# 3dlg-hcvc/tricolo

Hardware: AMD Instinct MI355X
Metric: trimodal training samples/sec (32^3 voxel + 6-view) (higher is better)
Workload: dtype f16 (f16 activation storage + f16 MFMA operands, fp32 accumulate; bf16x3 heads/GRU; within 1e-3 of the fp32 reference)

## Files before the change

include/tricolo_hip.h:

```cpp
#ifndef TRICOLO_HIP_H
#define TRICOLO_HIP_H
#include <stddef.h>
#include <stdint.h>

#ifdef __cplusplus
extern "C" {
#endif

#define TRI_FMT_F32 0
#define TRI_FMT_BF16 1
#define TRI_FMT_F16 2

int tri_version(void);
const char* tri_last_error(void);

typedef struct TriConvDesc {
    int B, ID, IH, IW, Cin;
    int OD, OH, OW, Cout;
    int KD, KH, KW, stride, pad_d, pad_h, pad_w;
} TriConvDesc;

int tri_conv_kpad(int ntaps, int cin_stored);
typedef struct TriPrepDesc {
    const float* w;
    void* hi;
    void* lo;
    long s_row, s_tap, s_inner;
    int rows, ntaps, inner, inner_pad, kpad, fmt;
    int frag;
} TriPrepDesc;
int tri_weight_prep_multi(const TriPrepDesc* descs_dev, int n, void* stream);
int tri_weight_prep(const float* w, long s_row, long s_tap, long s_inner, int rows, int ntaps, int inner, int inner_pad,
                    void* w_hi, void* w_lo, int fmt, int frag, void* stream);

int tri_embedding_fwd(const int* tokens, const float* weight, int B, int L, int D, float* out, void* stream);
int tri_embedding_bwd(const int* tokens, const float* dout, int B, int L, int V, int D, int padding_idx, float* dweight, void* stream);

int tri_retrieval_topk(const float* text, const float* shape, const int* label, int Nq, int Ns, int D, int k, int* topk_idx ,
                       double* topk_sim , int* first_hit , void* stream);

int tri_linear_small_supported(int M, int K, int N);
int tri_linear_small_fwd(const float* x, const float* w, const float* bias, float* y, int M, int K, int N, int act, int split3, void* stream);
int tri_linear_small_dgrad(const float* dout, const float* y, const float* w, float* dx, int M, int K, int N, int act, int split3,
                           void* stream);
int tri_linear_small_wgrad(const float* x, const float* dout, const float* y, float* dw, float* db , int M, int K, int N,
                           int act, int split3, void* stream);
int tri_linear_small_bwd(const float* x, const float* dout, const float* y, const float* w, float* dx, float* dw, float* db, int M, int K,
                         int N, int act, int split3, void* stream);

int tri_conv_num_mtiles(const TriConvDesc* d, int split3);
int tri_conv_num_records(const TriConvDesc* d, int split3, int row_list);
int tri_conv_kernel_family(const TriConvDesc* d, int transposed, int split3);
int tri_conv_wgrad_kernel_family(const TriConvDesc* d, int act_fmt);
size_t tri_conv_workspace(const TriConvDesc* d, int transposed);
int tri_conv_fwd(const TriConvDesc* d, const void* in, const void* w_hi, const void* w_lo, void* out, const uint8_t* row_mask,
                 const float* bias, int act, int accumulate, float* stats, int act_fmt, void* workspace, size_t workspace_bytes,
                 const int* row_pos , const int* row_count ,
                 void* stream);
int tri_conv_dgrad(const TriConvDesc* d, const void* dout, const void* wt_hi, const void* wt_lo, void* din, const uint8_t* row_mask,
                   int accumulate, int act_fmt, void* workspace, size_t workspace_bytes,
                   const int* row_pos ,
                   const int* row_count ,
                   void* stream);
typedef struct TriConvBnSums {
    const void* y;
    const float* relu_scale;
    const float* relu_shift;
    const void* relu_out;
    float* partial;
} TriConvBnSums;
int tri_conv_dgrad_bn_records(const TriConvDesc* d, int accumulate, int act_fmt);
int tri_conv_dgrad_bn(const TriConvDesc* d, const void* dout, const void* wt_hi, const void* wt_lo, void* din, int accumulate,
                      int act_fmt, void* workspace, size_t workspace_bytes, const int* row_pos, const TriConvBnSums* sums, void* stream);
size_t tri_conv_wgrad_workspace(const TriConvDesc* d);
size_t tri_conv_plan_bytes(const TriConvDesc* d);
int tri_conv_plan_build(const TriConvDesc* d, void* plan, void* stream);
int tri_conv_wgrad(const TriConvDesc* d, const void* in, const void* dout, const uint8_t* row_mask, const void* plan ,
                   void* workspace, size_t workspace_bytes, float* dw, long s_co, long s_tap, long s_ci, int cin_real, int split3,
                   int act_fmt, float out_scale ,
                   const int* row_pos, const int* row_count ,
                   void* stream);
#ifndef TRI_WGRAD_GROUP_MAX
#define TRI_WGRAD_GROUP_MAX 24
#endif
typedef struct TriWgradReduce {
    const float* slab;
// ... 173 lines not shown
```

tricolo_amd/_C.py:

```python
from __future__ import annotations

import ctypes as C
import os

import torch

_HERE = os.path.dirname(os.path.abspath(__file__))
LIB_PATH = os.path.join(_HERE, "libtricolo_hip.so")


class TriConvDesc(C.Structure):
    _fields_ = [(n, C.c_int) for n in ("B", "ID", "IH", "IW", "Cin", "OD", "OH", "OW", "Cout",
                                       "KD", "KH", "KW", "stride", "pad_d", "pad_h", "pad_w")]


class TriPrepDesc(C.Structure):
    _fields_ = [("w", C.c_void_p), ("hi", C.c_void_p), ("lo", C.c_void_p), ("s_row", C.c_long), ("s_tap", C.c_long),
                ("s_inner", C.c_long), ("rows", C.c_int), ("ntaps", C.c_int), ("inner", C.c_int), ("inner_pad", C.c_int),
                ("kpad", C.c_int), ("fmt", C.c_int), ("frag", C.c_int)]


class TriWgradReduce(C.Structure):
    _fields_ = [("slab", C.c_void_p), ("dw", C.c_void_p), ("s_co", C.c_long), ("s_tap", C.c_long), ("s_ci", C.c_long)] + \
               [(n, C.c_int) for n in ("splits", "Cout", "Kpad", "ntaps", "cin_stored", "cin_real", "zlanes", "nblocks")] + \
# ... 5 lines not shown
                ("workspace_bytes", C.c_size_t), ("dw", C.c_void_p), ("s_co", C.c_long), ("s_tap", C.c_long), ("s_ci", C.c_long),
                ("cin_real", C.c_int), ("out_scale", C.c_float), ("row_pos", C.c_void_p), ("row_count", C.c_void_p)]


class TriConvBnSums(C.Structure):
    _fields_ = [("y", C.c_void_p), ("relu_scale", C.c_void_p), ("relu_shift", C.c_void_p), ("relu_out", C.c_void_p), ("partial", C.c_void_p)]


TRI_WGRAD_JOBS_MAX = 12
TRI_ERR_ARG, TRI_ERR_UNSUPPORTED = -1, -2

P, I, L, F, Z, DBL = C.c_void_p, C.c_int, C.c_long, C.c_float, C.c_size_t, C.c_double
DP = C.POINTER(TriConvDesc)

SIGNATURES = {
    "tri_version": (I, []),
    "tri_last_error": (C.c_char_p, []),
    "tri_conv_kpad": (I, [I, I]),
    "tri_weight_prep": (I, [P, L, L, L, I, I, I, I, P, P, I, I, P]),
    "tri_weight_prep_multi": (I, [P, I, P]),
    "tri_embedding_fwd": (I, [P, P, I, I, I, P, P]),
    "tri_embedding_bwd": (I, [P, P, I, I, I, I, I, P, P]),
    "tri_retrieval_topk": (I, [P, P, P, I, I, I, I, P, P, P, P]),
    "tri_linear_small_supported": (I, [I, I, I]),
    "tri_linear_small_fwd": (I, [P, P, P, P, I, I, I, I, I, P]),
    "tri_linear_small_dgrad": (I, [P, P, P, P, I, I, I, I, I, P]),
    "tri_linear_small_wgrad": (I, [P, P, P, P, P, I, I, I, I, I, P]),
    "tri_linear_small_bwd": (I, [P, P, P, P, P, P, P, I, I, I, I, I, P]),
    "tri_conv_num_mtiles": (I, [DP, I]),
    "tri_conv_num_records": (I, [DP, I, I]),
    "tri_conv_workspace": (Z, [DP, I]),
    "tri_conv_kernel_family": (I, [DP, I, I]),
    "tri_conv_wgrad_kernel_family": (I, [DP, I]),
    "tri_conv_fwd": (I, [DP, P, P, P, P, P, P, I, I, P, I, P, Z, P, P, P]),
    "tri_conv_dgrad": (I, [DP, P, P, P, P, P, I, I, P, Z, P, P, P]),
    "tri_conv_dgrad_bn_records": (I, [DP, I, I]),
    "tri_conv_dgrad_bn": (I, [DP, P, P, P, P, I, I, P, Z, P, C.POINTER(TriConvBnSums), P]),
    "tri_conv_wgrad_workspace": (Z, [DP]),
    "tri_conv_plan_bytes": (Z, [DP]),
    "tri_conv_plan_build": (I, [DP, P, P]),
    "tri_conv_wgrad": (I, [DP, P, P, P, P, P, Z, P, L, L, L, I, I, I, F, P, P, P]),
    "tri_conv_wgrad_partial": (I, [DP, P, P, P, P, P, Z, P, L, L, L, I, I, I, F, P, P, P, P]),
    "tri_wgrad_reduce_grouped": (I, [P, I, P]),
    "tri_wgrad_reduce_grouped_noted": (I, [P, I, P, P]),
    "tri_conv_stem_wgrad_bn": (I, [DP, P, P, P, P, P, P, P, P, P, P, Z, P, L, L, L, I, I, F, P, P]),
    "tri_conv_wgrad_group_info": (I, [DP, I, P, P, P]),
    "tri_conv_wgrad_partial_group": (I, [P, I, I, P, P]),
    "tri_bn_finalize": (I, [P, I, I, P, I, P, P, P, P, P, F, F, P, P, P, P, P]),
    "tri_bn_eval_coeffs": (I, [I, P, P, P, P, F, P, P, P, P, P]),
    "tri_bn_act": (I, [P, P, P, P, P, P, P, L, I, I, I, P]),
    "tri_relu_bwd": (I, [P, P, P, L, I, P]),
    "tri_bn_bwd_num_blocks": (I, [L]),
    "tri_bn_bwd_reduce": (I, [P, P, L, I, P, P, P, P, P, I, P]),
    "tri_bn_bwd_finalize": (I, [P, I, I, P, I, P, P, P, P, P, P, P, P, F, P]),
    "tri_bn_bwd_small": (I, [P, P, L, I, P, I, P, P, P, P, P, P, P, P, I, P, P, P, F, I, P]),
    "tri_bn_bwd_apply": (I, [P, P, P, P, P, P, P, L, I, P, P, P, P, I, I, P]),
    "tri_bn_bwd_pair_reduce": (I, [P, P, P, P, L, I, P, P, I, P]),
    "tri_bn_bwd_pair_finalize": (I, [P, P, I, I, I, P, P, P, P, P, P, P, P, F, P]),
    "tri_bn_bwd_pair_apply": (I, [P, P, P, P, P, P, P, P, P, L, I, I, P]),
    "tri_bn_relu_pool3d_fwd": (I, [P, P, P, P, I, I, I, P, P, I, P]),
    "tri_pool3d_bwd_route": (I, [P, P, P, P, P, P, I, I, I, P, I, P]),
    "tri_pool3d_bwd_route_rows": (I, [P, P, P, P, P, P, I, I, I, P, P, P, I, P]),
    "tri_pool3d_bwd_route_rows_num_blocks": (I, [I, I, I]),
    "tri_pool3d_bwd_route_rows_reduce": (I, [P, P, P, P, P, P, I, I, I, P, P, P, P, I, P]),
    "tri_bn_bwd_apply_rows": (I, [P, P, P, P, P, P, I, P, P, L, I, P]),
    "tri_bn_bwd_rows_scratch": (C.c_size_t, [I]),
# ... 129 lines not shown
```

tricolo_amd/csrc/conv_wgrad.hip:

```cpp
#include "common.h"
#include <stdio.h>
#include <stdlib.h>
#include "../../include/tricolo_hip.h"
#include "conv_vox.h"

struct WgradArgs {
    const void* in;
    const void* dout;
    const uint8_t* row_mask;
    const int* row_pos;
    const int* row_count;
    float* slab;
    const int* plan_off;
    const unsigned* plan_mask;
    unsigned in_bytes;
    int B, ID, IH, IW, Cin;
    int OD, OH, OW, Cout;
    int KD, KH, KW, stride, pd, ph, pw;
    int Kpad, M, ntaps, cin_shift, steps_per_split, ntiles, nsplits;
    int plan_ring;
    FastDiv dOW, dOH, dOD, dCin;
#ifdef WGRAD_STAMPS
    long long* dbg;
#endif
// ... 889 lines not shown
                const int p0 = pc0 + toff, p1 = pc1 + toff;
                s16x4 lo = __builtin_amdgcn_ds_read_tr16_b64_v4i16((s16x4 __attribute__((address_space(3)))*)(slab + p0 * 128 + ((cq ^ (p0 & 3)) << 5) + fp * 8));
                s16x4 hi = __builtin_amdgcn_ds_read_tr16_b64_v4i16((s16x4 __attribute__((address_space(3)))*)(slab + p1 * 128 + ((cq ^ (p1 & 3)) << 5) + fp * 8));
                typedef short s16x8 __attribute__((ext_vector_type(8)));
                const s16x8 rr = {lo[0], lo[1], lo[2], lo[3], hi[0], hi[1], hi[2], hi[3]};
                const v8 bf = __builtin_bit_cast(v8, rr);
#pragma unroll
                for (int ct = 0; ct < 4; ++ct) acc[j][ct] = MM::mma(af[ct], bf, acc[j][ct]);
            }
            xx0 += 32; while (xx0 >= W) { xx0 -= W; ++rr0; }
            xx1 += 32; while (xx1 >= W) { xx1 -= W; ++rr1; }
        }
    }
    float* out = p.slab + (size_t)blockIdx.x * 64 * 576;
#pragma unroll
    for (int j = 0; j < 9; ++j) {
        const int nt = wave + 4 * j;
        const int k0 = (nt >> 2) * 64 + (nt & 3) * 16;
#pragma unroll
        for (int ct = 0; ct < 4; ++ct)
#pragma unroll
            for (int r = 0; r < 4; ++r) out[(size_t)(ct * 16 + fg * 4 + r) * 576 + k0 + fr] = acc[j][ct][r];
    }
}

struct KrowArgs {
    const void* in; const void* dout; float* slab;
    unsigned in_bytes, dout_bytes;
    int NH, H, W, Cin, Cout, Kpad;
    int Hin, Win;
    int rps, P, npiece;
    int nsteps, steps_per_split, nsplits, ntiles, ci_chunks;
    FastDiv dH, dP, dW;
};
struct KrowJobs {
    KrowArgs d[WGRAD_JOBS_MAX];
    int first_block[WGRAD_JOBS_MAX + 1];
    int n;
};
static_assert(sizeof(KrowJobs) <= 4096, "the job table travels in the kernel arguments (4 KB)");
#define KROW_SLAB_PX 96
#define KROW_SLAB_PX_S2 160
__device__ __forceinline__ int krow_sw(int r, int xs, int W) {
    const int hb = W > 8 ? (xs >> 3) & 1 : (W > 4 ? r & 1 : (r >> 1) & 1);
    return ((xs >> 1) & 1) | (hb << 1);
}
template <int CO_T, typename E, int S = 1>
__global__ __launch_bounds__(256, 2) void conv_wgrad_krow_kernel(const KrowJobs jobs) {
    typedef Mma<E> MM;
    typedef typename MM::v8 v8;
    constexpr int KB = 64;
    constexpr int XROW = CO_T * 2, X_BYTES = KB * XROW;
    constexpr int SLAB_BYTES = (S == 1 ? KROW_SLAB_PX : KROW_SLAB_PX_S2) * 128, STAGE = X_BYTES + SLAB_BYTES;
    constexpr int NSP = SLAB_BYTES / 4096;
    constexpr int XRPI = 1024 / XROW, XNI = KB / (4 * XRPI);
    constexpr int TM = CO_T / 32;
    static_assert((4 * XRPI) % 16 == 0 && XNI >= 1, "lane -> chunk map must not depend on the instruction");
    extern __shared__ __attribute__((aligned(16))) char smem[];
    int ji = 0;
    while (ji + 1 < jobs.n && (int)blockIdx.x >= jobs.first_block[ji + 1]) ++ji;
    const KrowArgs& p = jobs.d[ji];
    const int bid = (int)blockIdx.x - jobs.first_block[ji];
    const int t = threadIdx.x, lane = t & 63, wave = __builtin_amdgcn_readfirstlane(t >> 6);
    const int ntiles = p.ntiles;
    int split, tile;
    if (p.nsplits >= 16) {
        const int grp = bid / (8 * ntiles), rem = bid - grp * 8 * ntiles;
        split = grp * 8 + (rem & 7);
        tile = rem >> 3;
    } else {
        const int nb = p.nsplits * ntiles;
        if (bid >= nb) return;
        const int lid = xcd_remap(bid, nb);
        split = lid / ntiles;
        tile = lid - split * ntiles;
    }
    if (split >= p.nsplits) return;
    const int ky = tile % 3, rest = tile / 3;
    const int cic = rest % p.ci_chunks, cot = rest / p.ci_chunks;
    const int co0 = cot * CO_T, ci0 = cic * 64;
    const int ks_begin = split * p.steps_per_split, ks_end = min(p.nsteps, ks_begin + p.steps_per_split);
    const int W = p.W, P = p.P, H = p.H, Cin = p.Cin, Cout = p.Cout;
    const int st = S ? S : (p.Hin != p.H ? 2 : 1);
    const int wi = wave >> 1, wj = wave & 1;
    const int fr = lane & 15, fg = lane >> 4, fqq = fr >> 2, fp = fr & 3;

    const int xrow0 = wave * XRPI + lane / (XROW / 16), xsl = lane % (XROW / 16);
    const int xchunk = ((((xsl >> 1) ^ nat_sw<XROW>(xrow0)) & (XROW / 32 - 1)) << 1) | (xsl & 1);
    const unsigned xoff = (unsigned)((xrow0 * Cout + co0 + xchunk * 8) * 2);
    const unsigned xstep = (unsigned)(4 * XRPI * Cout * 2);
    const unsigned step_bytes = (unsigned)(p.rps * W) * (unsigned)(Cout * 2);
    int s_r[NSP], s_col[NSP];
#pragma unroll
    for (int i = 0; i < NSP; ++i) {
        const int pi = wave + 4 * i;
// ... 72 lines not shown
        }
    };

    if (ks_begin < ks_end) {
        issue_x(ks_begin, 0);
        issue_slab(ks_begin, 0);
        int buf = 0;
        for (int ks = ks_begin; ks < ks_end; ++ks) {
            asm volatile("s_waitcnt vmcnt(0)" ::: "memory");
            __builtin_amdgcn_s_barrier();
            asm volatile("" ::: "memory");
            const bool more = ks + 1 < ks_end;
            if (more) issue_x(ks + 1, buf ^ 1);
#pragma unroll
            for (int h = 0; h < 2; ++h) {
                if (h == 1 && more) issue_slab(ks + 1, buf ^ 1);
                compute(buf, h);
            }
            buf ^= 1;
        }
    }
    float* slab = p.slab + (size_t)split * Cout * p.Kpad;
#pragma unroll
    for (int a = 0; a < TM; ++a)
#pragma unroll
        for (int r = 0; r < 4; ++r) {
            const int co = co0 + wi * (CO_T / 2) + a * 16 + fg * 4 + r;
#pragma unroll
            for (int b = 0; b < 6; ++b) {
                const int tt = 6 * wj + b, kx = tt >> 2, cq = tt & 3;
                slab[(size_t)co * p.Kpad + (ky * 3 + kx) * Cin + ci0 + cq * 16 + fr] = acc[a][b][r];
            }
        }
}

__device__ __forceinline__ unsigned wgrad_nonfinite(float x) { return (__float_as_uint(x) & 0x7f800000u) == 0x7f800000u ? 1u : 0u; }
__device__ __forceinline__ void wgrad_note_bad(unsigned bad, int* note) {
    if (note && __any(bad) && (threadIdx.x & 63) == 0) atomicMax(note + 2, note[0] + note[3] + 1);
}
__device__ __forceinline__ void wgrad_reduce_block(const float* __restrict__ slab, int splits, int Cout, int Kpad, int ntaps, int cin_stored,
                                                   int cin_real, float* __restrict__ dw, long s_co, long s_tap, long s_ci, int zlanes,
                                                   float out_scale, unsigned block, float4* part, unsigned& bad, int kw_real = 0,
                                                   int kw_shift = 3) {
    const int kq = 256 / zlanes;
    const int ql = threadIdx.x % kq, zl = threadIdx.x / kq;
    const int K4 = (ntaps * cin_stored) >> 2;
    const long quad = (long)block * kq + ql;
    const bool live = quad < (long)Cout * K4;
    const int co = live ? (int)(quad / K4) : 0, k = live ? (int)(quad - (long)co * K4) * 4 : 0;
    float4 s = make_float4(0.f, 0.f, 0.f, 0.f);
    if (live) {
        const float* src = slab + (size_t)co * Kpad + k;
        const size_t zs = (size_t)Cout * Kpad;
#pragma unroll 4
        for (int z = zl; z < splits; z += zlanes) {
            float4 v = *(const float4*)(src + z * zs);
            s.x += v.x; s.y += v.y; s.z += v.z; s.w += v.w;
        }
    }
    part[threadIdx.x] = s;
    __syncthreads();
    if (zl == 0 && live) {
        for (int z = 1; z < zlanes; ++z) {
            float4 v = part[z * kq + ql];
            s.x += v.x; s.y += v.y; s.z += v.z; s.w += v.w;
        }
// ... 215 lines not shown
    static int per_cu = -1;
    if (per_cu < 0) per_cu = 2;
    *grid = tri_internal_num_cus() * (per_cu < 1 ? 1 : per_cu);
    if (*grid > g->ntiles) *grid = g->ntiles;
    return true;
}

static bool krow_geometry(const TriConvDesc* d, int act_fmt, KrowArgs* g, int* co_t, int* tiles, int* steps) {
    if (!act_fmt || krow_wgrad_disabled()) return false;
    if (d->KD != 1 || d->ID != 1 || d->KH != 3 || d->KW != 3 || (d->stride != 1 && d->stride != 2) || d->pad_d != 0 || d->pad_h != 1 || d->pad_w != 1) return false;
    if (d->Cin % 64 || d->Cout % 64 || d->OH * d->stride != d->IH || d->OW * d->stride != d->IW) return false;
    const int W = d->OW, H = d->OH;
    if (W < 4 || W > 64) return false;
    const size_t in_bytes = (size_t)d->B * d->IH * d->IW * d->Cin * 2, dout_bytes = (size_t)d->B * H * W * d->Cout * 2;
    if (in_bytes >= ((size_t)1 << 31) || dout_bytes >= ((size_t)1 << 31)) return false;
    KrowArgs a{};
    a.in_bytes = (unsigned)in_bytes; a.dout_bytes = (unsigned)dout_bytes;
    a.NH = d->B * H; a.H = H; a.W = W; a.Cin = d->Cin; a.Cout = d->Cout; a.Kpad = 9 * d->Cin;
    a.Hin = d->IH; a.Win = d->IW;
    a.rps = 64 / W;
    a.P = d->stride == 1 ? ((W + 3) & ~1) : 2 * W + 2;
    if (a.rps * a.P > (d->stride == 1 ? KROW_SLAB_PX : KROW_SLAB_PX_S2)) return false;
    a.npiece = (a.rps * a.P + 7) / 8;
    a.nsteps = (a.NH + a.rps - 1) / a.rps;
    a.ci_chunks = d->Cin / 64;
    *co_t = d->Cout % 128 == 0 ? 128 : 64;
    a.ntiles = (d->Cout / *co_t) * 3 * a.ci_chunks;
    a.dH = make_fastdiv(H); a.dP = make_fastdiv(a.P); a.dW = make_fastdiv(W);
    *g = a;
    *tiles = a.ntiles;
    *steps = a.nsteps;
    return true;
}
#define KROW_TARGET_BLOCKS 512
static void krow_plan_alone(int tiles, int steps, int* sps, int* splits) {
    int s = KROW_TARGET_BLOCKS / tiles;
    const int max_by_steps = steps / 4 > 0 ? steps / 4 : 1;
    if (s > max_by_steps) s = max_by_steps;
    if (s < 1) s = 1;
    if (s > 1024) s = 1024;
    *sps = (steps + s - 1) / s;
    *splits = (steps + *sps - 1) / *sps;
}
static inline int krow_blocks(const KrowArgs& a) {
    return a.nsplits >= 16 ? ((a.nsplits + 7) / 8) * 8 * a.ntiles : (a.nsplits * a.ntiles + 7) / 8 * 8;
}
template <int CO_T, typename E, int S>
static int launch_krow_jobs(const KrowArgs* a, int n, hipStream_t stream) {
    constexpr int STAGE = 64 * CO_T * 2 + (S == 1 ? KROW_SLAB_PX : KROW_SLAB_PX_S2) * 128;
    KrowJobs jobs{};
    int order[WGRAD_JOBS_MAX];
    for (int i = 0; i < n; ++i) order[i] = i;
    for (int i = 1; i < n; ++i)
        for (int j = i; j > 0 && a[order[j]].steps_per_split > a[order[j - 1]].steps_per_split; --j) { int t = order[j]; order[j] = order[j - 1]; order[j - 1] = t; }
    int blocks = 0;
    for (int i = 0; i < n; ++i) {
        jobs.d[i] = a[order[i]];
        jobs.first_block[i] = blocks;
        blocks += krow_blocks(a[order[i]]);
    }
    jobs.first_block[n] = blocks;
    jobs.n = n;
    static bool attr_set = false;
    if (!attr_set) {
        hipFuncSetAttribute((const void*)conv_wgrad_krow_kernel<CO_T, E, S>, hipFuncAttributeMaxDynamicSharedMemorySize, 2 * STAGE);
        attr_set = true;
    }
    conv_wgrad_krow_kernel<CO_T, E, S><<<dim3(blocks), 256, 2 * STAGE, stream>>>(jobs);
    return tri_check_launch("tri_conv_wgrad(krow)");
}
static int launch_krow(int co_t, int act_fmt, const KrowArgs* a, int n, hipStream_t s) {
    int n2 = 0;
    for (int i = 0; i < n; ++i) n2 += a[i].Hin != a[i].H;
    if (n2 && n2 != n) {
#define TRI_KR0 (act_fmt == TRI_FMT_F16 ? (co_t == 128 ? launch_krow_jobs<128, f16_t, 0>(a, n, s) : launch_krow_jobs<64, f16_t, 0>(a, n, s))   \
                                        : (co_t == 128 ? launch_krow_jobs<128, bf16_t, 0>(a, n, s) : launch_krow_jobs<64, bf16_t, 0>(a, n, s)))
        return TRI_KR0;
#undef TRI_KR0
    }
    const bool s2 = n2 > 0;
#define TRI_KR(S_)                                                                                                                      \
    (act_fmt == TRI_FMT_F16 ? (co_t == 128 ? launch_krow_jobs<128, f16_t, S_>(a, n, s) : launch_krow_jobs<64, f16_t, S_>(a, n, s))      \
                            : (co_t == 128 ? launch_krow_jobs<128, bf16_t, S_>(a, n, s) : launch_krow_jobs<64, bf16_t, S_>(a, n, s)))
    return s2 ? TRI_KR(2) : TRI_KR(1);
#undef TRI_KR
}

extern "C" size_t tri_conv_wgrad_workspace(const TriConvDesc* d) {
    size_t need = 0;
    {
        StemWgradArgs sg; int grid;
        if (stem_wgrad_geometry(d, 1, &sg, &grid)) need = (size_t)grid * 64 * d->KH * 32 * sizeof(float);
        C64WgradArgs cg;
        if (c64_wgrad_geometry(d, 1, &cg, &grid)) need = (size_t)grid * 64 * 576 * sizeof(float);
        TriVox0Geom vg;
        if (tri_internal_vox0_geometry(d->B, d->ID, d->IH, d->IW, d->Cin, d->OD, d->OH, d->OW, d->Cout, d->KD, d->KH, d->KW, d->stride, d->pad_d,
                                       d->pad_h, d->pad_w, &vg) && tri_internal_vox0_wgrad_grid(vg) > 0)
            need = (size_t)tri_internal_vox0_wgrad_grid(vg) * 32 * 144 * sizeof(float);
        KrowArgs kg; int co_t, tiles, steps;
        if (krow_geometry(d, 1, &kg, &co_t, &tiles, &steps)) {
            int sps, splits;
            krow_plan_alone(tiles, steps, &sps, &splits);
            const size_t n = (size_t)splits * d->Cout * kg.Kpad * sizeof(float);
            if (n > need) need = n;
        }
    }
    for (int mode = 0; mode < 4; ++mode) {
        int BI, BJ, tiles, splits, sps, Kpad, dma;
        wgrad_plan(d, mode & 1, mode >> 1, &BI, &BJ, &tiles, &splits, &sps, &Kpad, &dma);
        size_t n = (size_t)splits * d->Cout * Kpad * sizeof(float);
        if (n > need) need = n;
    }
    return need;
}

extern "C" int tri_conv_wgrad_kernel_family(const TriConvDesc* d, int act_fmt) {
    {
        TriVox0Geom vg;
        if (act_fmt && tri_internal_vox0_geometry(d->B, d->ID, d->IH, d->IW, d->Cin, d->OD, d->OH, d->OW, d->Cout, d->KD, d->KH, d->KW, d->stride,
                                                  d->pad_d, d->pad_h, d->pad_w, &vg) && tri_internal_vox0_wgrad_grid(vg) > 0)
            return 6;
    }
    {
        C64WgradArgs cg; KrowArgs kg; int grid, co_t, tiles, steps;
        if (!c64_wgrad_geometry(d, act_fmt, &cg, &grid) && krow_geometry(d, act_fmt, &kg, &co_t, &tiles, &steps)) return 7;
    }
    int BI, BJ, tiles, splits, sps, Kpad, dma;
    wgrad_plan(d, act_fmt, 0, &BI, &BJ, &tiles, &splits, &sps, &Kpad, &dma);
    return dma ? 2 : 0;
}

static inline int wgrad_dma_blocks(const WgradArgs& a) {
    return a.nsplits >= 16 ? ((a.nsplits + 7) / 8) * 8 * a.ntiles : a.nsplits * a.ntiles;
}
static inline size_t wgrad_dma_plan_bytes(const WgradArgs& a) {
    const size_t entries = a.plan_ring ? (size_t)2 * WGRAD_RING_STEPS * 64 : (size_t)a.steps_per_split * 64;
    return entries * (a.row_count ? 12 : 8);
}
template <int BI, int BJ, typename E, int NWI = 2, int NWJ = 2>
static int launch_wgrad_dma_jobs(const WgradArgs* a, int n, hipStream_t stream) {
    constexpr int STAGE = 64 * (BI * 2 + BJ * 2);
    WgradJobs jobs{};
    size_t plan_bytes = 0;
    int blocks = 0;
    for (int i = 0; i < n; ++i) {
        jobs.d[i] = a[i];
#ifdef WGRAD_STAMPS
        jobs.d[i].dbg = g_wgrad_dbg;
#endif
        jobs.first_block[i] = blocks;
        blocks += wgrad_dma_blocks(a[i]);
        if (wgrad_dma_plan_bytes(a[i]) > plan_bytes) plan_bytes = wgrad_dma_plan_bytes(a[i]);
    }
    jobs.first_block[n] = blocks;
    jobs.n = n;
    size_t smem = 2 * STAGE + 512 + plan_bytes;
#ifdef WGRAD_STAMPS
    smem += 2048;
#endif
    static bool attr_set = false;
    if (!attr_set) {
        hipFuncSetAttribute((const void*)conv_wgrad_dma_kernel<BI, BJ, E, NWI, NWJ>, hipFuncAttributeMaxDynamicSharedMemorySize,
// ... 167 lines not shown
    {
        TriVox0Geom vg; int grid;
        if (row_mask && !row_count && !split3 && act_fmt &&
            tri_internal_vox0_geometry(d->B, d->ID, d->IH, d->IW, d->Cin, d->OD, d->OH, d->OW, d->Cout, d->KD, d->KH, d->KW, d->stride, d->pad_d,
                                       d->pad_h, d->pad_w, &vg) && (grid = tri_internal_vox0_wgrad_grid(vg)) > 0) {
            const size_t need = (size_t)grid * 32 * 144 * sizeof(float);
            if (workspace_bytes < need) { tri_set_error("wgrad(vox0): workspace too small"); return TRI_ERR_ARG; }
            int rc = tri_internal_vox0_wgrad_launch(vg, grid, d->B, in, dout, row_mask, (float*)workspace, act_fmt, (hipStream_t)stream);
            if (rc) return rc;
            const long quads = (long)32 * 36;
            int zlanes = 1;
            while (zlanes < 64 && zlanes * 2 <= grid && quads * zlanes < 262144) zlanes *= 2;
            const int kq = 256 / zlanes;
            pending->slab = (const float*)workspace; pending->dw = dw; pending->s_co = s_co; pending->s_tap = s_tap; pending->s_ci = s_ci;
            pending->splits = grid; pending->Cout = 32; pending->Kpad = 144; pending->ntaps = 36; pending->cin_stored = 4;
            pending->cin_real = cin_real; pending->zlanes = zlanes; pending->nblocks = (int)((quads + kq - 1) / kq);
            pending->out_scale = out_scale; pending->kw_real = 3; pending->kw_shift = 2;
            return 0;
        }
    }
    {
        StemWgradArgs sg; int grid;
        if (!row_mask && !row_count && !split3 && stem_wgrad_geometry(d, act_fmt, &sg, &grid)) {
            sg.in = in; sg.dout = dout;
            sg.y = nullptr;
            return stem_wgrad_launch(d, sg, grid, workspace, workspace_bytes, dw, s_co, s_tap, s_ci, cin_real, act_fmt, out_scale, pending, stream);
        }
    }
    if (d->Cin % 4 != 0 || d->Cout % 4 != 0) { tri_set_error("wgrad: channels must be multiples of 4"); return TRI_ERR_ARG; }
    {
        KrowArgs kg; int co_t, tiles, steps;
        if (!row_mask && !row_count && !split3 && krow_geometry(d, act_fmt, &kg, &co_t, &tiles, &steps)) {
            int sps, splits;
            krow_plan_alone(tiles, steps, &sps, &splits);
            if (workspace_bytes < (size_t)splits * d->Cout * kg.Kpad * sizeof(float)) { tri_set_error("wgrad(krow): workspace too small"); return TRI_ERR_ARG; }
            kg.in = in; kg.dout = dout; kg.slab = (float*)workspace; kg.steps_per_split = sps; kg.nsplits = splits;
            int rc = launch_krow(co_t, act_fmt, &kg, 1, (hipStream_t)stream);
            if (rc) return rc;
            wgrad_fill_pending(d, (const float*)workspace, splits, kg.Kpad, dw, s_co, s_tap, s_ci, cin_real, out_scale, pending);
            return 0;
        }
    }
    int BI, BJ, tiles, splits, sps, Kpad, dma;
    wgrad_plan(d, act_fmt, row_count != nullptr, &BI, &BJ, &tiles, &splits, &sps, &Kpad, &dma);
    if (workspace_bytes < (size_t)splits * d->Cout * Kpad * sizeof(float)) { tri_set_error("wgrad: workspace too small"); return TRI_ERR_ARG; }
    WgradArgs a{};
    {
        int rc = wgrad_fill_args(d, in, dout, row_mask, plan, (float*)workspace, row_pos, row_count, split3, act_fmt, Kpad, sps, tiles, splits, &a);
        if (rc) return rc;
    }
    hipStream_t s = (hipStream_t)stream;
    int rc;
#define TRI_WG(BI_, BJ_)                                                                                   \
    (act_fmt == TRI_FMT_F16 ? launch_wgrad<BI_, BJ_, 1, f16_t>(a, tiles, splits, s)                      \
     : act_fmt == TRI_FMT_BF16 ? launch_wgrad<BI_, BJ_, 1, bf16_t>(a, tiles, splits, s)                  \
              : (split3 ? launch_wgrad<BI_, BJ_, 2, float>(a, tiles, splits, s) : launch_wgrad<BI_, BJ_, 1, float>(a, tiles, splits, s)))
    if (dma) {
        if ((size_t)a.M * a.Cout * 2 >= ((size_t)1 << 31)) { tri_set_error("wgrad: dOut tensor >= 2 GiB (32-bit buffer offsets)"); return TRI_ERR_UNSUPPORTED; }
        if (act_fmt == TRI_FMT_F16) rc = BI == 128 ? launch_wgrad_dma<128, 128, f16_t>(a, tiles, splits, s) : launch_wgrad_dma<64, 128, f16_t>(a, tiles, splits, s);
        else rc = BI == 128 ? launch_wgrad_dma<128, 128, bf16_t>(a, tiles, splits, s) : launch_wgrad_dma<64, 128, bf16_t>(a, tiles, splits, s);
    } else if (BI == 128) rc = TRI_WG(128, 128);
    else if (BJ == 256) rc = TRI_WG(64, 256);
    else rc = TRI_WG(64, 128);
#undef TRI_WG
    if (rc) return rc;
    wgrad_fill_pending(d, (const float*)workspace, splits, Kpad, dw, s_co, s_tap, s_ci, cin_real, out_scale, pending);
    return 0;
}

static bool wgrad_wide_tiles() {
// ... 17 lines not shown
        KrowArgs kg; int co_t;
        if (krow_geometry(d, act_fmt, &kg, &co_t, tiles, steps)) { *family = co_t == 128 ? 4 : (d->stride == 2 ? 7 : 5); return 0; }
    }
    int BI, BJ, t, splits, sps, Kpad, dma;
    wgrad_plan(d, act_fmt, 0, &BI, &BJ, &t, &splits, &sps, &Kpad, &dma);
    if (!dma) return 0;
    *family = BI == 128 ? 1 : 2;
    if (BI == 128 && d->Cout % 256 == 0 && wgrad_wide_tiles()) {
        *family = 3;
        t = (d->Cout / 256) * ((Kpad + 127) / 128);
    }
    *tiles = t;
    *steps = (int)(((long)d->B * d->OD * d->OH * d->OW + 63) / 64);
    return 0;
}
extern "C" int tri_conv_wgrad_partial_group(const TriWgradJob* jobs, int n, int act_fmt, TriWgradReduce* pending, void* stream) {
    if (n < 1 || n > WGRAD_JOBS_MAX || !jobs || !pending) { tri_set_error("wgrad group: 1..TRI_WGRAD_JOBS_MAX jobs"); return TRI_ERR_ARG; }
    static_assert(WGRAD_JOBS_MAX == TRI_WGRAD_JOBS_MAX, "header and kernel disagree");
    {
        int fam, t0, st0;
        tri_conv_wgrad_group_info(jobs[0].d, act_fmt, &fam, &t0, &st0);
        if (fam >= 4 && fam <= 7) {
            KrowArgs ka[WGRAD_JOBS_MAX];
            int co_t0 = 0, tl[WGRAD_JOBS_MAX], st[WGRAD_JOBS_MAX];
            long total = 0;
            for (int i = 0; i < n; ++i) {
                int co_t;
                if (jobs[i].row_pos || jobs[i].row_count || !krow_geometry(jobs[i].d, act_fmt, &ka[i], &co_t, &tl[i], &st[i]) || (i && co_t != co_t0)) {
                    tri_set_error("wgrad group: jobs must share one groupable kernel family"); return TRI_ERR_ARG;
                }
                co_t0 = co_t;
                total += (long)tl[i] * st[i];
            }
            int common = (int)((total + wgrad_group_target(fam) - 1) / wgrad_group_target(fam));
            if (common < 8) common = 8;
            for (int i = 0; i < n; ++i) {
                int sps_alone, splits_alone;
                krow_plan_alone(tl[i], st[i], &sps_alone, &splits_alone);
                int sps = n == 1 ? sps_alone : (common > sps_alone ? common : sps_alone);
                if (sps > st[i]) sps = st[i];
                const int splits = (st[i] + sps - 1) / sps;
                sps = (st[i] + splits - 1) / splits;
                const TriConvDesc* d = jobs[i].d;
                if (jobs[i].workspace_bytes < (size_t)splits * d->Cout * ka[i].Kpad * sizeof(float)) { tri_set_error("wgrad group(krow): workspace too small"); return TRI_ERR_ARG; }
                ka[i].in = jobs[i].in; ka[i].dout = jobs[i].dout; ka[i].slab = (float*)jobs[i].workspace;
                ka[i].steps_per_split = sps; ka[i].nsplits = splits;
                wgrad_fill_pending(d, (const float*)jobs[i].workspace, splits, ka[i].Kpad, jobs[i].dw, jobs[i].s_co, jobs[i].s_tap, jobs[i].s_ci,
                                   jobs[i].cin_real, jobs[i].out_scale, &pending[i]);
            }
            return launch_krow(co_t0, act_fmt, ka, n, (hipStream_t)stream);
        }
    }
    WgradArgs a[WGRAD_JOBS_MAX];
    int fam0 = 0, ind_sps[WGRAD_JOBS_MAX], tiles[WGRAD_JOBS_MAX], steps[WGRAD_JOBS_MAX], Kpads[WGRAD_JOBS_MAX];
    long total = 0;
    for (int i = 0; i < n; ++i) {
        int fam;
        tri_conv_wgrad_group_info(jobs[i].d, act_fmt, &fam, &tiles[i], &steps[i]);
        if (!fam || (i && fam != fam0)) { tri_set_error("wgrad group: jobs must share one groupable kernel family"); return TRI_ERR_ARG; }
        fam0 = fam;
        int BI, BJ, t, splits, dma;
        wgrad_plan(jobs[i].d, act_fmt, 0, &BI, &BJ, &t, &splits, &ind_sps[i], &Kpads[i], &dma);
        total += (long)tiles[i] * steps[i];
    }
    const int target = wgrad_group_target(fam0);
    int common = (int)((total + target - 1) / target);
    if (common < 1) common = 1;
    for (;; ++common) {
        long wgs = 0;
        for (int i = 0; i < n; ++i) {
            const int sps = common > ind_sps[i] ? common : ind_sps[i];
            wgs += (long)tiles[i] * ((steps[i] + sps - 1) / sps);
        }
        if (wgs <= target || common >= 4096) break;
    }
    for (int i = 0; i < n; ++i) {
        int sps = (n == 1 && fam0 != 3) ? ind_sps[i] : (common > ind_sps[i] ? common : ind_sps[i]);
        if (sps > steps[i]) sps = steps[i];
        const int splits = (steps[i] + sps - 1) / sps;
        if (n > 1 || fam0 == 3) sps = (steps[i] + splits - 1) / splits;
        const TriConvDesc* d = jobs[i].d;
        if (jobs[i].workspace_bytes < (size_t)splits * d->Cout * Kpads[i] * sizeof(float)) { tri_set_error("wgrad group: workspace too small"); return TRI_ERR_ARG; }
        if ((size_t)d->B * d->OD * d->OH * d->OW * d->Cout * 2 >= ((size_t)1 << 31)) { tri_set_error("wgrad: dOut tensor >= 2 GiB (32-bit buffer offsets)"); return TRI_ERR_UNSUPPORTED; }
// ... 51 lines not shown
```

tricolo_amd/ops.py:

```python
from __future__ import annotations

import math
import os

import torch

from . import _C
from ._C import check, lib, make_desc, ptr, stream

_PRECISIONS = ("bf16", "bf16x3", "f16")
_FMT = {torch.float32: 0, torch.bfloat16: 1, torch.float16: 2}
F16_GRAD_SCALE = float(os.environ.get("TRICOLO_F16_GRAD_SCALE", "4096"))
if not (F16_GRAD_SCALE >= 1.0 and math.frexp(F16_GRAD_SCALE)[0] == 0.5):
    raise ValueError(f"TRICOLO_F16_GRAD_SCALE={F16_GRAD_SCALE!r}: must be a power of two >= 1 (the kernels divide it out exactly)")
_default_precision = os.environ.get("TRICOLO_PRECISION", "bf16x3")


def set_default_precision(p: str):
    global _default_precision
    if p not in _PRECISIONS:
        raise ValueError(f"precision must be one of {_PRECISIONS}")
    _default_precision = p


# ... 145 lines not shown
    return 1 if lo is not None else (2 if x.dtype != torch.float32 else 0)


_FRAG_FAMILIES = (13, 14, 15)


class ConvGeom:

    def __init__(self, B, in_grid, cin, cin_stored, cout, kernel, stride, pad, weight_strides):
        ID, IH, IW = in_grid
        KD, KH, KW = kernel
        pd, ph, pw = pad
        OD = (ID + 2 * pd - KD) // stride + 1
        OH = (IH + 2 * ph - KH) // stride + 1
        OW = (IW + 2 * pw - KW) // stride + 1
        self.B, self.in_grid, self.out_grid = B, (ID, IH, IW), (OD, OH, OW)
        self.cin, self.cin_stored, self.cout = cin, cin_stored, cout
        self.kernel, self.stride, self.pad = kernel, stride, pad
        self.ntaps = KD * KH * KW
        self.strides = weight_strides
        self.desc = make_desc(B, ID, IH, IW, cin_stored, OD, OH, OW, cout, KD, KH, KW, stride, pd, ph, pw)
        self.kpad = lib().tri_conv_kpad(self.ntaps, cin_stored)
        self.kpad_t = lib().tri_conv_kpad(self.ntaps, cout)
        self.M = B * OD * OH * OW
        self.M_in = B * ID * IH * IW
        self.num_mtiles = {m: lib().tri_conv_num_mtiles(_C.C.byref(self.desc), m) for m in (0, 1, 2)}
        self.num_records_rows = {m: lib().tri_conv_num_records(_C.C.byref(self.desc), m, 1) for m in (0, 1, 2)}
        self.kernel_family = {(tr, m): lib().tri_conv_kernel_family(_C.C.byref(self.desc), 1 if tr else 0, m)
                              for tr in (False, True) for m in (0, 1, 2)}
        self.wgrad_ws = lib().tri_conv_wgrad_workspace(_C.C.byref(self.desc))
        fam = lib().tri_conv_wgrad_kernel_family(_C.C.byref(self.desc), 1)
        self.wgrad_dma = fam == 2
        self.wgrad_krow = fam == 7
        self.wgrad_brick = fam == 6
        self._plans = {}
        self.fwd_ws = lib().tri_conv_workspace(_C.C.byref(self.desc), 0)
        self.dgrad_ws = lib().tri_conv_workspace(_C.C.byref(self.desc), 1) if cin == cin_stored and cin % 32 == 0 else 0

    def dgrad_row_order(self, device):
        if self.stride != 2 or self.ntaps == 1:
            return None
        t = self._plans.get(("rowpos", device))
        if t is None:
            ID, IH, IW = self.in_grid
            pd, ph, pw = self.pad
            pos = torch.arange(self.M_in, dtype=torch.int64)
            x, r = pos % IW, pos // IW
            y, r = r % IH, r // IH
            z = r % ID
            cls = (((z + pd) & 1) << 2) | (((y + ph) & 1) << 1) | ((x + pw) & 1)
            order = torch.sort(cls * self.M_in + pos).indices
            t = order.to(torch.int32).to(device)
            self._plans[("rowpos", device)] = t
        return t

    def brick(self, transposed: bool, mode: int) -> bool:
        return (self.kernel_family[(transposed, mode)] & 255) in (6, 7, 13, 14)

    def packed_frag(self, transposed: bool, precision: str, storage=None) -> int:
        storage = storage or act_dtype(precision)
        mode = 1 if precision == "bf16x3" else (2 if storage != torch.float32 else 0)
        return 1 if (self.kernel_family[(transposed, mode)] & 255) in _FRAG_FAMILIES else 0

    def check_packed(self, packed, transposed: bool, x):
        need = 1 if (self.kernel_family[(transposed, _conv_mode(x, packed[1]))] & 255) in _FRAG_FAMILIES else 0
        if getattr(packed[0], "tri_frag", 0) != need:
# ... 292 lines not shown
            self.ci, self.off, self.descs = 0, 0, []
            self.dws.clear()
            return
        early, ev, last = self._pre
        self._pre = None
        late, self.descs = self.descs, []
        self.launch_jobs(last)
        with torch.cuda.stream(side.fork(event=ev)):
            self._reduce(early)
        side.join()
        self._reduce(late + self.descs)
        self.ci, self.off, self.descs = 0, 0, []
        self.dws.clear()


def wgrad_batch(device):
    return WgradBatch(device) if _WGRAD_GROUPED else None


def conv_wgrad(x, dout, g: ConvGeom, like: torch.Tensor, precision: str, row_mask=None, out_scale: float = 1.0, batch=None, rows=None):
    assert rows is None or row_mask is None
    assert x.dtype == dout.dtype
    dw = torch.empty_like(like)
    ws = batch.slab(g.wgrad_ws) if batch is not None else _workspace(g.wgrad_ws, x.device)
    plan = g.plan(x.device)
    s_co, s_tap, s_ci = g.strides
    bi = 128 if (g.cout % 128 == 0 and g.kpad >= 128) else 64
    h16 = x.dtype != torch.float32
    bj = 128 if bi == 128 else (256 if (g.kpad <= 256 and not (h16 and g.wgrad_dma)) else 128)
    s3 = 1 if (split3(precision) and not h16) else 0
    if h16 and g.wgrad_brick and row_mask is not None:
        sym = f"conv_vox0_wgrad_kernel<{_TNAME[x.dtype]}>"
    elif h16 and g.wgrad_krow and row_mask is None and rows is None:
        sym = f"conv_wgrad_krow_kernel<{128 if g.cout % 128 == 0 else 64}, {_TNAME[x.dtype]}>"
    elif h16 and g.wgrad_dma:
        sym = f"conv_wgrad_dma_kernel<{bi}, {bj}, {_TNAME[x.dtype]}>"
    else:
        sym = f"conv_wgrad_kernel<{bi}, {bj}, {2 if s3 else 1}, {_TNAME[x.dtype]}>"
    if batch is not None and batch.group_jobs and h16 and row_mask is None:
        fam, tiles, _ = g.wgrad_group(_abf(x))
        if fam:
            xa, da = _act(x), _act(dout)
            job = _C.TriWgradJob(_C.C.pointer(g.desc), ptr(xa), ptr(da), ptr(plan), ptr(ws), ws.numel(), ptr(dw), s_co, s_tap, s_ci, g.cin,
                                 float(out_scale), ptr(rows[0]) if rows else None, ptr(rows[1]) if rows else None)
            batch.add_job(fam, tiles, job, (xa, da, ws, dw, plan, rows), _flops(g, rows), sym)
            batch.dws[dw.data_ptr()] = dw
            return dw
    if batch is not None:
        batch.dws[dw.data_ptr()] = dw
        desc = _C.TriWgradReduce()
        check(_timed(sym, _flops(g, rows, row_mask),
                     lambda: lib().tri_conv_wgrad_partial(_C.C.byref(g.desc), ptr(_act(x)), ptr(_act(dout)), ptr(row_mask), ptr(plan),
                                                          ptr(ws), ws.numel(), ptr(dw), s_co, s_tap, s_ci, g.cin, s3, _abf(x),
                                                          float(out_scale), ptr(rows[0]) if rows else None,
                                                          ptr(rows[1]) if rows else None, _C.C.byref(desc), stream())),
              "tri_conv_wgrad_partial")
        batch.descs.append(desc)
        return dw
    check(_timed(sym, _flops(g, rows, row_mask),
                 lambda: lib().tri_conv_wgrad(_C.C.byref(g.desc), ptr(_act(x)), ptr(_act(dout)), ptr(row_mask), ptr(plan), ptr(ws),
                                              ws.numel(), ptr(dw), s_co, s_tap, s_ci, g.cin, s3, _abf(x), float(out_scale),
                                              ptr(rows[0]) if rows else None, ptr(rows[1]) if rows else None, stream())),
          "tri_conv_wgrad")
    return dw


class BNCoeffs:
# ... 711 lines not shown
```

Measured before the change: 12900.

## Add k-block wgrad kernel form for small-width stride-1 convs

Adds a new wgrad kernel body (kblock) for stride-1 convs with small spatial width. It stages a multi-row input slab with halo rows in LDS and computes all nine taps for a 64-channel tile from it, and makes tile counts and split planning aware of this form. The row-based krow body is factored out so one kernel can serve mixed job groups. The aim is better reuse of input rows across taps and more parallel tiles for small-grid layers. The cost is more register pressure (9 taps times TM accumulators), a larger LDS footprint, and a changed grouping target.

Result: no change. 12990 (median of 6 runs) (+0.7%).

```diff
diff --git a/include/tricolo_hip.h b/include/tricolo_hip.h
--- a/include/tricolo_hip.h
+++ b/include/tricolo_hip.h
@@ -52,6 +52,7 @@
 int tri_conv_num_records(const TriConvDesc* d, int split3, int row_list);
 int tri_conv_kernel_family(const TriConvDesc* d, int transposed, int split3);
 int tri_conv_wgrad_kernel_family(const TriConvDesc* d, int act_fmt);
+int tri_conv_wgrad_krow_form(const TriConvDesc* d, int act_fmt);
 size_t tri_conv_workspace(const TriConvDesc* d, int transposed);
 int tri_conv_fwd(const TriConvDesc* d, const void* in, const void* w_hi, const void* w_lo, void* out, const uint8_t* row_mask,
                  const float* bias, int act, int accumulate, float* stats, int act_fmt, void* workspace, size_t workspace_bytes,
diff --git a/tricolo_amd/_C.py b/tricolo_amd/_C.py
--- a/tricolo_amd/_C.py
+++ b/tricolo_amd/_C.py
@@ -61,6 +61,7 @@
     "tri_conv_workspace": (Z, [DP, I]),
     "tri_conv_kernel_family": (I, [DP, I, I]),
     "tri_conv_wgrad_kernel_family": (I, [DP, I]),
+    "tri_conv_wgrad_krow_form": (I, [DP, I]),
     "tri_conv_fwd": (I, [DP, P, P, P, P, P, P, I, I, P, I, P, Z, P, P, P]),
     "tri_conv_dgrad": (I, [DP, P, P, P, P, P, I, I, P, Z, P, P, P]),
     "tri_conv_dgrad_bn_records": (I, [DP, I, I]),
diff --git a/tricolo_amd/csrc/conv_wgrad.hip b/tricolo_amd/csrc/conv_wgrad.hip
--- a/tricolo_amd/csrc/conv_wgrad.hip
+++ b/tricolo_amd/csrc/conv_wgrad.hip
@@ -945,6 +945,8 @@
     int rps, P, npiece;
     int nsteps, steps_per_split, nsplits, ntiles, ci_chunks;
     FastDiv dH, dP, dW;
+    int form, hh, srows;
+    FastDiv dHH, dHH2;
 };
 struct KrowJobs {
     KrowArgs d[WGRAD_JOBS_MAX];
@@ -958,8 +960,8 @@
     const int hb = W > 8 ? (xs >> 3) & 1 : (W > 4 ? r & 1 : (r >> 1) & 1);
     return ((xs >> 1) & 1) | (hb << 1);
 }
-template <int CO_T, typename E, int S = 1>
-__global__ __launch_bounds__(256, 2) void conv_wgrad_krow_kernel(const KrowJobs jobs) {
+template <int CO_T, typename E, int S>
+__device__ __forceinline__ void krow_row_body(const KrowArgs& p, const int bid) {
     typedef Mma<E> MM;
     typedef typename MM::v8 v8;
     constexpr int KB = 64;
@@ -970,10 +972,6 @@
     constexpr int TM = CO_T / 32;
     static_assert((4 * XRPI) % 16 == 0 && XNI >= 1, "lane -> chunk map must not depend on the instruction");
     extern __shared__ __attribute__((aligned(16))) char smem[];
-    int ji = 0;
-    while (ji + 1 < jobs.n && (int)blockIdx.x >= jobs.first_block[ji + 1]) ++ji;
-    const KrowArgs& p = jobs.d[ji];
-    const int bid = (int)blockIdx.x - jobs.first_block[ji];
     const int t = threadIdx.x, lane = t & 63, wave = __builtin_amdgcn_readfirstlane(t >> 6);
     const int ntiles = p.ntiles;
     int split, tile;
@@ -1112,6 +1110,167 @@
                 slab[(size_t)co * p.Kpad + (ky * 3 + kx) * Cin + ci0 + cq * 16 + fr] = acc[a][b][r];
             }
         }
+}
+
+template <int CO_T, typename E, int S = 1>
+__global__ __launch_bounds__(256, 2) void conv_wgrad_krow_kernel(const KrowJobs jobs) {
+    int ji = 0;
+    while (ji + 1 < jobs.n && (int)blockIdx.x >= jobs.first_block[ji + 1]) ++ji;
+    krow_row_body<CO_T, E, S>(jobs.d[ji], (int)blockIdx.x - jobs.first_block[ji]);
+}
+
+#define KBLK_SLAB_PX 160
+template <typename E>
+__device__ __forceinline__ void kblock_body(const KrowArgs& p, const int bid) {
+    typedef Mma<E> MM;
+    typedef typename MM::v8 v8;
+    constexpr int CO_T = 64, KB = 64;
+    constexpr int XROW = CO_T * 2, X_BYTES = KB * XROW;
+    constexpr int SLAB_BYTES = KBLK_SLAB_PX * 128, STAGE = X_BYTES + SLAB_BYTES;
+    constexpr int NSP = SLAB_BYTES / 4096;
+    constexpr int XRPI = 1024 / XROW, XNI = KB / (4 * XRPI);
+    constexpr int TM = CO_T / 16;
+    extern __shared__ __attribute__((aligned(16))) char smem[];
+    const int t = threadIdx.x, lane = t & 63, wave = __builtin_amdgcn_readfirstlane(t >> 6);
+    const int ntiles = p.ntiles;
+    int split, tile;
+    if (p.nsplits >= 16) {
+        const int grp = bid / (8 * ntiles), rem = bid - grp * 8 * ntiles;
+        split = grp * 8 + (rem & 7);
+        tile = rem >> 3;
+    } else {
+        const int nb = p.nsplits * ntiles;
+        if (bid >= nb) return;
+        const int lid = xcd_remap(bid, nb);
+        split = lid / ntiles;
+        tile = lid - split * ntiles;
+    }
+    if (split >= p.nsplits) return;
+    const int cot = tile / p.ci_chunks, cic = tile - cot * p.ci_chunks;
+    const int co0 = cot * CO_T, ci0 = cic * 64;
+    const int ks_begin = split * p.steps_per_split, ks_end = min(p.nsteps, ks_begin + p.steps_per_split);
+    const int W = p.W, P = p.P, H = p.H, Cin = p.Cin, Cout = p.Cout, hh = p.hh;
+    const int fr = lane & 15, fg = lane >> 4, fqq = fr >> 2, fp = fr & 3;
+
+    const int xrow0 = wave * XRPI + lane / (XROW / 16), xsl = lane % (XROW / 16);
+    const int xchunk = ((((xsl >> 1) ^ nat_sw<XROW>(xrow0)) & (XROW / 32 - 1)) << 1) | (xsl & 1);
+    const unsigned xoff = (unsigned)((xrow0 * Cout + co0 + xchunk * 8) * 2);
+    const unsigned xstep = (unsigned)(4 * XRPI * Cout * 2);
+    const unsigned step_bytes = (unsigned)(p.rps * W) * (unsigned)(Cout * 2);
+    int s_gj[NSP], s_col[NSP];
+#pragma unroll
+    for (int i = 0; i < NSP; ++i) {
+        const int pi = wave + 4 * i;
+        const int q = 8 * pi + (lane >> 3), c = lane & 7;
+        const int r = (int)fdiv((uint32_t)q, p.dP), xs = q - r * P;
+        const int g = (int)fdiv((uint32_t)r, p.dHH2);
+        const int cq = ((c >> 1) ^ krow_sw(r, xs, W)) & 3;
+        s_gj[i] = ((g * hh) << 8) | (r - g * (hh + 2));
+        s_col[i] = (xs >= 1 && xs <= W && r < p.srows) ? ((xs - 1) * Cin + ci0 + cq * 16 + (c & 1) * 8) * 2 : -1;
+    }
+    unsigned boff[2][9];
+#pragma unroll
+    for (int h = 0; h < 2; ++h)
+#pragma unroll
+        for (int hf = 0; hf < 2; ++hf) {
+            const int pos = 32 * h + 8 * fg + 4 * hf + fqq;
+            const int r = (int)fdiv((uint32_t)pos, p.dW), x = pos - r * W;
+            const int g = (int)fdiv((uint32_t)r, p.dHH);
+            const int sr0 = r + 2 * g;
+#pragma unroll
+            for (int tap = 0; tap < 9; ++tap) {
+                const int ky = tap / 3, kx = tap - 3 * ky;
+                const int sr = sr0 + ky, xs = x + kx;
+                const unsigned o = (unsigned)((sr * P + xs) * 128 + (((wave ^ krow_sw(sr, xs, W)) & 3) << 5) + fp * 8);
+                boff[h][tap] = hf ? boff[h][tap] | (o << 16) : o;
+            }
+        }
+
+    f32x4 acc[TM][9];
+#pragma unroll
+    for (int a = 0; a < TM; ++a)
+#pragma unroll
+        for (int b = 0; b < 9; ++b) acc[a][b] = (f32x4){0.f, 0.f, 0.f, 0.f};
+
+    const v4i rsrc = make_rsrc_words(p.in, p.in_bytes);
+    const v4i xrsrc = make_rsrc_words(p.dout, p.dout_bytes);
+    const unsigned lds0 = lds_addr(smem) + wave * 1024;
+    const int row_bytes = W * Cin * 2;
+
+    auto issue_x = [&](int ks, int buf) {
+        const unsigned xb = lds0 + buf * STAGE;
+        const unsigned xbase = xoff + (unsigned)ks * step_bytes;
+#pragma unroll
+        for (int i = 0; i < XNI; ++i) dma16_async(xrsrc, xb + i * 4096, (int)(xbase + i * xstep));
+    };
+    auto issue_slab = [&](int ks, int buf) {
+        const unsigned sb = lds0 + buf * STAGE + X_BYTES;
+        int vo[NSP];
+#pragma unroll
+        for (int i = 0; i < NSP; ++i) {
+            const int G = ks * p.rps + (s_gj[i] >> 8), j = (s_gj[i] & 255) - 1;
+            const int n = (int)fdiv((uint32_t)G, p.dH), yy = G - n * H + j;
+            const bool ok = s_col[i] >= 0 && G < p.NH && (unsigned)yy < (unsigned)H;
+            vo[i] = ok ? (G + j) * row_bytes + s_col[i] : (int)0x80000000;
+        }
+#pragma unroll
+        for (int i = 0; i < NSP; ++i)
+            if (wave + 4 * i < p.npiece) dma16_async(rsrc, sb + i * 4096, vo[i]);
+    };
+    auto compute = [&](int buf, int h) {
+        const char* xb = smem + buf * STAGE + h * 32 * XROW;
+        const char* sb = smem + buf * STAGE + X_BYTES;
+        v8 af[TM];
+#pragma unroll
+        for (int a = 0; a < TM; ++a) af[a] = tr_frag<XROW, v8>(xb, a * 16, fg, fqq, fp);
+#pragma unroll
+        for (int b = 0; b < 9; ++b) {
+            s16x4 lo = __builtin_amdgcn_ds_read_tr16_b64_v4i16((s16x4 __attribute__((address_space(3)))*)(sb + (boff[h][b] & 0xffffu)));
+            s16x4 hi = __builtin_amdgcn_ds_read_tr16_b64_v4i16((s16x4 __attribute__((address_space(3)))*)(sb + (boff[h][b] >> 16)));
+            typedef short s16x8 __attribute__((ext_vector_type(8)));
+            const s16x8 rr = {lo[0], lo[1], lo[2], lo[3], hi[0], hi[1], hi[2], hi[3]};
+            const v8 bf = __builtin_bit_cast(v8, rr);
+#pragma unroll
+            for (int a = 0; a < TM; ++a) acc[a][b] = MM::mma(af[a], bf, acc[a][b]);
+        }
+    };
+
+    if (ks_begin < ks_end) {
+        issue_x(ks_begin, 0);
+        issue_slab(ks_begin, 0);
+        int buf = 0;
+        for (int ks = ks_begin; ks < ks_end; ++ks) {
+            asm volatile("s_waitcnt vmcnt(0)" ::: "memory");
+            __builtin_amdgcn_s_barrier();
+            asm volatile("" ::: "memory");
+            const bool more = ks + 1 < ks_end;
+            if (more) issue_x(ks + 1, buf ^ 1);
+#pragma unroll
+            for (int h = 0; h < 2; ++h) {
+                if (h == 1 && more) issue_slab(ks + 1, buf ^ 1);
+                compute(buf, h);
+            }
+            buf ^= 1;
+        }
+    }
+    float* slab = p.slab + (size_t)split * Cout * p.Kpad;
+#pragma unroll
+    for (int a = 0; a < TM; ++a)
+#pragma unroll
+        for (int r = 0; r < 4; ++r) {
+            const int co = co0 + a * 16 + fg * 4 + r;
+#pragma unroll
+            for (int b = 0; b < 9; ++b) slab[(size_t)co * p.Kpad + b * Cin + ci0 + wave * 16 + fr] = acc[a][b][r];
+        }
+}
+template <int CO_ROW, typename E>
+__global__ __launch_bounds__(256, 2) void conv_wgrad_kblock_kernel(const KrowJobs jobs) {
+    int ji = 0;
+    while (ji + 1 < jobs.n && (int)blockIdx.x >= jobs.first_block[ji + 1]) ++ji;
+    const KrowArgs& p = jobs.d[ji];
+    const int bid = (int)blockIdx.x - jobs.first_block[ji];
+    if (p.form) kblock_body<E>(p, bid);
+    else krow_row_body<CO_ROW, E, 0>(p, bid);
 }
 
 __device__ __forceinline__ unsigned wgrad_nonfinite(float x) { return (__float_as_uint(x) & 0x7f800000u) == 0x7f800000u ? 1u : 0u; }
@@ -1393,6 +1552,18 @@
     *steps = a.nsteps;
     return true;
 }
+static bool kblock_geometry(const TriConvDesc* d, KrowArgs* g) {
+    if (d->stride != 1 || g->W > 32 || 64 % g->W) return false;
+    const int H = g->H, rps = g->rps;
+    if (H % rps && rps % H) return false;
+    const int hh = H < rps ? H : rps, srows = (rps / hh) * (hh + 2);
+    if (srows * g->P > KBLK_SLAB_PX) return false;
+    g->form = 1; g->hh = hh; g->srows = srows;
+    g->npiece = (srows * g->P + 7) / 8;
+    g->ntiles = (d->Cout / 64) * g->ci_chunks;
+    g->dHH = make_fastdiv(hh); g->dHH2 = make_fastdiv(hh + 2);
+    return true;
+}
 #define KROW_TARGET_BLOCKS 512
 static void krow_plan_alone(int tiles, int steps, int* sps, int* splits) {
     int s = KROW_TARGET_BLOCKS / tiles;
@@ -1445,6 +1616,41 @@
                             : (co_t == 128 ? launch_krow_jobs<128, bf16_t, S_>(a, n, s) : launch_krow_jobs<64, bf16_t, S_>(a, n, s)))
     return s2 ? TRI_KR(2) : TRI_KR(1);
 #undef TRI_KR
+}
+
+template <int CO_ROW, typename E>
+static int launch_kblock_jobs(const KrowArgs* a, int n, hipStream_t stream) {
+    constexpr int STAGE_BLOCK = 64 * 64 * 2 + KBLK_SLAB_PX * 128, STAGE_ROW = 64 * CO_ROW * 2 + KROW_SLAB_PX_S2 * 128;
+    KrowJobs jobs{};
+    int order[WGRAD_JOBS_MAX];
+    for (int i = 0; i < n; ++i) order[i] = i;
+    for (int i = 1; i < n; ++i)
+        for (int j = i; j > 0 && a[order[j]].steps_per_split > a[order[j - 1]].steps_per_split; --j) { int t = order[j]; order[j] = order[j - 1]; order[j - 1] = t; }
+    int blocks = 0;
+    bool rows = false;
+    for (int i = 0; i < n; ++i) {
+        jobs.d[i] = a[order[i]];
+        jobs.first_block[i] = blocks;
+        blocks += krow_blocks(a[order[i]]);
+        rows |= !a[order[i]].form;
+    }
+    jobs.first_block[n] = blocks;
+    jobs.n = n;
+    static bool attr_set = false;
+    if (!attr_set) {
+        hipFuncSetAttribute((const void*)conv_wgrad_kblock_kernel<CO_ROW, E>, hipFuncAttributeMaxDynamicSharedMemorySize, 2 * (STAGE_ROW > STAGE_BLOCK ? STAGE_ROW : STAGE_BLOCK));
+        attr_set = true;
+    }
+    conv_wgrad_kblock_kernel<CO_ROW, E><<<dim3(blocks), 256, 2 * (rows && STAGE_ROW > STAGE_BLOCK ? STAGE_ROW : STAGE_BLOCK), stream>>>(jobs);
+    return tri_check_launch("tri_conv_wgrad(kblock)");
+}
+static int launch_kblock(int co_row, int act_fmt, const KrowArgs* a, int n, hipStream_t s) {
+    if (act_fmt == TRI_FMT_F16) return co_row == 128 ? launch_kblock_jobs<128, f16_t>(a, n, s) : launch_kblock_jobs<64, f16_t>(a, n, s);
+    return co_row == 128 ? launch_kblock_jobs<128, bf16_t>(a, n, s) : launch_kblock_jobs<64, bf16_t>(a, n, s);
+}
+static int krow_choose_form(const TriConvDesc* d, KrowArgs* g) {
+    kblock_geometry(d, g);
+    return g->ntiles;
 }
 
 extern "C" size_t tri_conv_wgrad_workspace(const TriConvDesc* d) {
@@ -1461,7 +1667,7 @@
         KrowArgs kg; int co_t, tiles, steps;
         if (krow_geometry(d, 1, &kg, &co_t, &tiles, &steps)) {
             int sps, splits;
-            krow_plan_alone(tiles, steps, &sps, &splits);
+            krow_plan_alone(krow_choose_form(d, &kg), steps, &sps, &splits);
             const size_t n = (size_t)splits * d->Cout * kg.Kpad * sizeof(float);
             if (n > need) need = n;
         }
@@ -1489,6 +1695,13 @@
     int BI, BJ, tiles, splits, sps, Kpad, dma;
     wgrad_plan(d, act_fmt, 0, &BI, &BJ, &tiles, &splits, &sps, &Kpad, &dma);
     return dma ? 2 : 0;
+}
+
+extern "C" int tri_conv_wgrad_krow_form(const TriConvDesc* d, int act_fmt) {
+    if (tri_conv_wgrad_kernel_family(d, act_fmt) != 7) return 0;
+    KrowArgs kg; int co_t, tiles, steps;
+    if (!krow_geometry(d, act_fmt, &kg, &co_t, &tiles, &steps)) return 0;
+    return kblock_geometry(d, &kg) ? 2 : 1;
 }
 
 static inline int wgrad_dma_blocks(const WgradArgs& a) {
@@ -1722,10 +1935,10 @@
         KrowArgs kg; int co_t, tiles, steps;
         if (!row_mask && !row_count && !split3 && krow_geometry(d, act_fmt, &kg, &co_t, &tiles, &steps)) {
             int sps, splits;
-            krow_plan_alone(tiles, steps, &sps, &splits);
+            krow_plan_alone(krow_choose_form(d, &kg), steps, &sps, &splits);
             if (workspace_bytes < (size_t)splits * d->Cout * kg.Kpad * sizeof(float)) { tri_set_error("wgrad(krow): workspace too small"); return TRI_ERR_ARG; }
             kg.in = in; kg.dout = dout; kg.slab = (float*)workspace; kg.steps_per_split = sps; kg.nsplits = splits;
-            int rc = launch_krow(co_t, act_fmt, &kg, 1, (hipStream_t)stream);
+            int rc = kg.form ? launch_kblock(co_t, act_fmt, &kg, 1, (hipStream_t)stream) : launch_krow(co_t, act_fmt, &kg, 1, (hipStream_t)stream);
             if (rc) return rc;
             wgrad_fill_pending(d, (const float*)workspace, splits, kg.Kpad, dw, s_co, s_tap, s_ci, cin_real, out_scale, pending);
             return 0;
@@ -1809,11 +2022,14 @@
                 co_t0 = co_t;
                 total += (long)tl[i] * st[i];
             }
-            int common = (int)((total + wgrad_group_target(fam) - 1) / wgrad_group_target(fam));
+            bool any_block = false;
+            for (int i = 0; i < n; ++i) { krow_choose_form(jobs[i].d, &ka[i]); any_block |= ka[i].form != 0; }
+            const int target = any_block ? KROW_TARGET_BLOCKS * 3 * 64 / co_t0 : wgrad_group_target(fam);
+            int common = (int)((total + target - 1) / target);
             if (common < 8) common = 8;
             for (int i = 0; i < n; ++i) {
                 int sps_alone, splits_alone;
-                krow_plan_alone(tl[i], st[i], &sps_alone, &splits_alone);
+                krow_plan_alone(ka[i].ntiles, st[i], &sps_alone, &splits_alone);
                 int sps = n == 1 ? sps_alone : (common > sps_alone ? common : sps_alone);
                 if (sps > st[i]) sps = st[i];
                 const int splits = (st[i] + sps - 1) / sps;
@@ -1825,7 +2041,7 @@
                 wgrad_fill_pending(d, (const float*)jobs[i].workspace, splits, ka[i].Kpad, jobs[i].dw, jobs[i].s_co, jobs[i].s_tap, jobs[i].s_ci,
                                    jobs[i].cin_real, jobs[i].out_scale, &pending[i]);
             }
-            return launch_krow(co_t0, act_fmt, ka, n, (hipStream_t)stream);
+            return any_block ? launch_kblock(co_t0, act_fmt, ka, n, (hipStream_t)stream) : launch_krow(co_t0, act_fmt, ka, n, (hipStream_t)stream);
         }
     }
     WgradArgs a[WGRAD_JOBS_MAX];
diff --git a/tricolo_amd/ops.py b/tricolo_amd/ops.py
--- a/tricolo_amd/ops.py
+++ b/tricolo_amd/ops.py
@@ -201,6 +201,7 @@
         fam = lib().tri_conv_wgrad_kernel_family(_C.C.byref(self.desc), 1)
         self.wgrad_dma = fam == 2
         self.wgrad_krow = fam == 7
+        self.wgrad_krow_form = lib().tri_conv_wgrad_krow_form(_C.C.byref(self.desc), 1)
         self.wgrad_brick = fam == 6
         self._plans = {}
         self.fwd_ws = lib().tri_conv_workspace(_C.C.byref(self.desc), 0)
@@ -559,7 +560,7 @@
     if h16 and g.wgrad_brick and row_mask is not None:
         sym = f"conv_vox0_wgrad_kernel<{_TNAME[x.dtype]}>"
     elif h16 and g.wgrad_krow and row_mask is None and rows is None:
-        sym = f"conv_wgrad_krow_kernel<{128 if g.cout % 128 == 0 else 64}, {_TNAME[x.dtype]}>"
+        sym = f"conv_wgrad_{'kblock' if g.wgrad_krow_form >= 2 else 'krow'}_kernel<{128 if g.cout % 128 == 0 else 64}, {_TNAME[x.dtype]}>"
     elif h16 and g.wgrad_dma:
         sym = f"conv_wgrad_dma_kernel<{bi}, {bj}, {_TNAME[x.dtype]}>"
     else:
```
